# joaobuibergen/roms-trunk-mgh

Hardware: AMD Instinct MI355X
Metric: simulated-days/wall-sec (higher is better)
Workload: dtype f64; 1 GPU; BENCHMARK3 2048x256x30 NT=2 nonlinear 3-D step incl. 59 step2d calls, U3/C4 tracer advection, analytic atmospheric forcing, bulk fluxes + KPP + diagnostics every step; tiling=1x1, halo_transport=none, rccl_ranks=0, graph_exchanges=1, ndtfast=20, finite=True

## Files before the change

roms_trunk_mgh_amd/csrc/k_step2d_mom.hip:

```cpp
#include "step2d_common.h"

namespace {

enum { RM_pm = 0, RM_pn, RM_on_u, RM_om_v, RM_fomn, RM_dndx, RM_dmde, RM_pmon_r, RM_pnom_r, RM_pmon_p, RM_pnom_p,
       RM_om_r, RM_on_r, RM_om_p, RM_on_p,
       RM_h, RM_visc2_r, RM_visc2_p, RM_COUNT };
#define RM_FIRST_GROUP RM_h

typedef const double __attribute__((address_space(4))) *ccd_t;
template <bool ROWM>
struct Met {
  ccd_t tab;
  int nj, LBj;
  __device__ __forceinline__ double get(gcd_t A, int f, long q, int jr) const
  {
    if constexpr (ROWM) return tab[(jr - LBj) * RM_COUNT + f];
    else return A[q];
  }
};
#define MT(name, q, jr) met.get((gcd_t)c->F.name, RM_##name, (q), (jr))
#define HT(name, q, jr) meth.get((gcd_t)c->F.name, RM_##name, (q), (jr))

#define C6 (1.0 / 6.0)

struct T2 {
  const double *ub, *vb, *DU, *DV, *D;
  int i0, j0;
  int Istr, Iend, Jstr, Jend;
  bool s_edge, n_edge, w_edge, e_edge;
  __device__ __forceinline__ int at(int i, int j) const { return (i - i0) + (j - j0) * TP; }
};

__device__ __forceinline__ double UFx2(const T2 &m, int i, int j)
{
  int ia = i, ib = i + 1;
  if (m.w_edge) { if (ia == m.Istr) ia = m.Istr + 1; if (ib == m.Istr) ib = m.Istr + 1; }
  if (m.e_edge) { if (ia == m.Iend + 1) ia = m.Iend; if (ib == m.Iend + 1) ib = m.Iend; }
  const int a = m.at(i, j);
  return 0.25 * (m.ub[a] + m.ub[a + 1] - C6 * (d2x(m.ub, m.at(ia, j)) + d2x(m.ub, m.at(ib, j)))) *
         (m.DU[a] + m.DU[a + 1] - C6 * (d2x(m.DU, m.at(ia, j)) + d2x(m.DU, m.at(ib, j))));
}
__device__ __forceinline__ double UFe2(const T2 &m, int i, int j)
{
  int ja = j, jb = j - 1;
  if (m.s_edge) { if (ja == m.Jstr - 1) ja = m.Jstr; if (jb == m.Jstr - 1) jb = m.Jstr; }
  if (m.n_edge) { if (ja == m.Jend + 1) ja = m.Jend; if (jb == m.Jend + 1) jb = m.Jend; }
  const int a = m.at(i, j);
  return 0.25 * (m.ub[a] + m.ub[a - TP] - C6 * (d2y(m.ub, m.at(i, ja)) + d2y(m.ub, m.at(i, jb)))) *
         (m.DV[a] + m.DV[a - 1] - C6 * (d2x(m.DV, a) + d2x(m.DV, a - 1)));
}
__device__ __forceinline__ double VFx2(const T2 &m, int i, int j)
{
  int ia = i, ib = i - 1;
  if (m.w_edge) { if (ia == m.Istr - 1) ia = m.Istr; if (ib == m.Istr - 1) ib = m.Istr; }
  if (m.e_edge) { if (ia == m.Iend + 1) ia = m.Iend; if (ib == m.Iend + 1) ib = m.Iend; }
  const int a = m.at(i, j);
  return 0.25 * (m.vb[a] + m.vb[a - 1] - C6 * (d2x(m.vb, m.at(ia, j)) + d2x(m.vb, m.at(ib, j)))) *
         (m.DU[a] + m.DU[a - TP] - C6 * (d2y(m.DU, a) + d2y(m.DU, a - TP)));
}
__device__ __forceinline__ double VFe2(const T2 &m, int i, int j)
{
  int ja = j, jb = j + 1;
  if (m.s_edge) { if (ja == m.Jstr) ja = m.Jstr + 1; if (jb == m.Jstr) jb = m.Jstr + 1; }
  if (m.n_edge) { if (ja == m.Jend + 1) ja = m.Jend; if (jb == m.Jend + 1) jb = m.Jend; }
  const int a = m.at(i, j);
  return 0.25 * (m.vb[a] + m.vb[a + TP] - C6 * (d2y(m.vb, m.at(i, ja)) + d2y(m.vb, m.at(i, jb)))) *
         (m.DV[a] + m.DV[a + TP] - C6 * (d2y(m.DV, m.at(i, ja)) + d2y(m.DV, m.at(i, jb))));
}

__device__ __forceinline__ double UFx2_c2(const T2 &m, int a) { return 0.25 * (m.DU[a] + m.DU[a + 1]) * (m.ub[a] + m.ub[a + 1]); }
__device__ __forceinline__ double UFe2_c2(const T2 &m, int a) { return 0.25 * (m.DV[a] + m.DV[a - 1]) * (m.ub[a] + m.ub[a - TP]); }
__device__ __forceinline__ double VFx2_c2(const T2 &m, int a) { return 0.25 * (m.DU[a] + m.DU[a - TP]) * (m.vb[a] + m.vb[a - 1]); }
__device__ __forceinline__ double VFe2_c2(const T2 &m, int a) { return 0.25 * (m.DV[a] + m.DV[a + TP]) * (m.vb[a] + m.vb[a + TP]); }

template <bool FUSED, bool ROWM = false, bool ROWH = false, bool WET = false, bool C2 = false>
__global__ void __launch_bounds__(BLK_X *BLK_Y)
k2d_mom_lds(const RomsDev *__restrict__ c, S2 s, const double *__restrict__ DUon, const double *__restrict__ DVom,
            const double *__restrict__ zeta_new, const double *__restrict__ zwrk, double *__restrict__ DUnext,
            double *__restrict__ DVnext)
{
  DEV_PROLOGUE(c)
  const roms_params_t &p = c->p;
  const Met<ROWM> met{(ccd_t)c->rowm, (int)nj, LBj};
  const Met<ROWH> meth{(ccd_t)c->rowm, (int)nj, LBj};
  __shared__ double sU[TJ * TP], sV[TJ * TP], sDU[TJ * TP], sDV[TJ * TP], sD[TJ * TP];
  __shared__ double sZn[FUSED ? TJ * TP : 1], sZw[FUSED ? TJ * TP : 1];
  const bool img = FUSED && s.ew_images;
  const bool inline_bc = img || DUnext != nullptr;
  const Blk XB = xcd_block();
  const int i0 = b.Istr + XB.x * BLK_X, j0 = b.Jstr + XB.y * BLK_Y;
  static_assert(BLK_X == 64, "one wave per tile row");
  const int i = i0 + threadIdx.x, j = j0 + __builtin_amdgcn_readfirstlane(threadIdx.y);
  const gcd_t ubk = (gcd_t)(c->F.ubar + (long)(s.krhs - 1) * nij);
  const gcd_t vbk = (gcd_t)(c->F.vbar + (long)(s.krhs - 1) * nij);
  const gcd_t zk = (gcd_t)(c->F.zeta + (long)(s.krhs - 1) * nij);
  constexpr int ZW = BLK_X + 1, ZH = BLK_Y + 1;
  constexpr int ZIT = (ZW * ZH + BLK_X * BLK_Y - 1) / (BLK_X * BLK_Y);
  double z_zs[ZIT], z_zk[ZIT], z_rk[ZIT], z_rp[ZIT], z_rm[ZIT];
  double q_rhoA0 = 0.0, q_rhoS0 = 0.0, q_rhoAw = 0.0, q_rhoSw = 0.0, q_rhoAs = 0.0, q_rhoSs = 0.0;
  double q_zs0 = 0.0, q_zsw = 0.0, q_zss = 0.0, q_ruf = 0.0, q_rvf = 0.0, q_us = 0.0, q_vs = 0.0;
  double q_rubk = 0.0, q_rubp = 0.0, q_rvbk = 0.0, q_rvbp = 0.0;
  double q_Zt = 0.0, q_DU1 = 0.0, q_DU2 = 0.0, q_DV1 = 0.0, q_DV2 = 0.0, q_zkr = 0.0;
  if constexpr (FUSED) {
    const int tid = threadIdx.y * BLK_X + threadIdx.x;
    const gcd_t zsq = (gcd_t)(c->F.zeta + (long)(s.kstp - 1) * nij);
    const bool am3z = !(s.iif == 1 || s.predictor);
#pragma unroll
    for (int r = 0; r < ZIT; r++) {
      const int q = tid + r * BLK_X * BLK_Y;
      z_zs[r] = 0.0; z_zk[r] = 0.0; z_rk[r] = 0.0; z_rp[r] = 0.0; z_rm[r] = 1.0;
      if (q < ZW * ZH) {
        const int li = 1 + q % ZW, lj = 1 + q / ZW;
        int gi = i0 - 2 + li, gj = j0 - 2 + lj;
        if (img) gi = wrap_i(b, gi);
        else gi = gi < b.LBi ? b.LBi : (gi > b.UBi ? b.UBi : gi);
        gj = gj < b.LBj ? b.LBj : (gj > b.UBj ? b.UBj : gj);
        const long gq = I2(gi, gj);
        z_zs[r] = zsq[gq];
        z_zk[r] = zk[gq];
        if (am3z) {
          z_rk[r] = GF(rzeta)[gq + (long)(s.kstp - 1) * nij];
          z_rp[r] = GF(rzeta)[gq + (long)(3 - s.kstp - 1) * nij];
        }
        if (p.masking) z_rm[r] = GF(rmask)[gq];
      }
    }
    if (i <= b.Iend && j <= b.Jend) {
      const long a = I2(i, j);
      const gcd_t rhoA = (gcd_t)(c->F.rhoA), rhoS = (gcd_t)(c->F.rhoS);
      q_rhoA0 = rhoA[a]; q_rhoS0 = rhoS[a]; q_rhoAw = rhoA[a - 1]; q_rhoSw = rhoS[a - 1];
      q_rhoAs = rhoA[a - ni]; q_rhoSs = rhoS[a - ni];
      q_zs0 = zsq[a]; q_zsw = zsq[a - 1]; q_zss = zsq[a - ni];
      q_ruf = GF(rufrc)[a]; q_rvf = GF(rvfrc)[a];
      q_us = GF(ubar)[a + (long)(s.kstp - 1) * nij]; q_vs = GF(vbar)[a + (long)(s.kstp - 1) * nij];
      if (am3z) {
        q_rubk = GF(rubar)[a + (long)(s.kstp - 1) * nij]; q_rubp = GF(rubar)[a + (long)(3 - s.kstp - 1) * nij];
        q_rvbk = GF(rvbar)[a + (long)(s.kstp - 1) * nij]; q_rvbp = GF(rvbar)[a + (long)(3 - s.kstp - 1) * nij];
      }
      if (avg_reads_sums2(s)) { q_DU2 = GF(DU_avg2)[a]; q_DV2 = GF(DV_avg2)[a]; }
      if (avg_reads_sums1(s)) { q_Zt = GF(Zt_avg1)[a]; q_DU1 = GF(DU_avg1)[a]; q_DV1 = GF(DV_avg1)[a]; q_zkr = zk[a]; }
    }
  }
  {
    const int tid = threadIdx.y * BLK_X + threadIdx.x;
    for (int e = tid; e < TJ * TP; e += BLK_X * BLK_Y) {
      const int li = e % TP, lj = e / TP;
      int gi = i0 - 2 + li, gj = j0 - 2 + lj;
      if (img) gi = wrap_i(b, gi);
      else gi = gi < b.LBi ? b.LBi : (gi > b.UBi ? b.UBi : gi);
      gj = gj < b.LBj ? b.LBj : (gj > b.UBj ? b.UBj : gj);
      const long g = I2(gi, gj);
      const double ug = ubk[g], vg = vbk[g], Dg = zk[g] + HT(h, g, gj);
      sU[e] = ug;
      sV[e] = vg;
      sD[e] = Dg;
      if (DUon) {
        sDU[e] = DUon[g];
        sDV[e] = DVom[g];
      } else {
        sDU[e] = flux_u(ug, MT(on_u, g, gj), Dg, zk[g - 1] + HT(h, g - 1, gj));
        if (gj >= b.LBj + 1) sDV[e] = flux_v(vg, MT(om_v, g, gj), Dg, zk[g - ni] + HT(h, g - ni, gj - 1));
        else sDV[e] = 0.0;
      }
    }
  }
  __syncthreads();
  if constexpr (FUSED) {
    const int tid = threadIdx.y * BLK_X + threadIdx.x;
#pragma unroll
    for (int r = 0; r < ZIT; r++) {
      const int q = tid + r * BLK_X * BLK_Y;
      if (q < ZW * ZH) {
        const int li = 1 + q % ZW, lj = 1 + q / ZW;
        const int e = lj * TP + li;
        int gi = i0 - 2 + li, gj = j0 - 2 + lj;
        if (img) gi = wrap_i(b, gi);
        else gi = gi < b.LBi ? b.LBi : (gi > b.UBi ? b.UBi : gi);
        gj = gj < b.LBj ? b.LBj : (gj > b.UBj ? b.UBj : gj);
        const double rhs = (sDU[e] - sDU[e + 1]) + (sDV[e] - sDV[e + TP]);
        double zn, zw;
        const long gq = I2(gi, gj);
        zeta_step(p, s, rhs, MT(pm, gq, gj), MT(pn, gq, gj), z_zs[r], z_zk[r], z_rk[r], z_rp[r], z_rm[r],
                  p.masking != 0, zn, zw);
        sZn[e] = zn;
        sZw[e] = zw;
      }
    }
    __syncthreads();
  }
  if (i > b.Iend || j > b.Jend) return;
  auto put = [&](gd_t A, long idx, double val) {
    A[idx] = val;
    if (img) {
      if (i <= b.NghostPoints) A[idx + b.Lm] = val;
      if (i >= b.Lm - 2) A[idx - b.Lm] = val;
    }
  };
  const bool do_u = img || i >= b.IstrU;
  const bool do_v = j >= b.JstrV;
  const long a = I2(i, j);
  const gcd_t rhoA = (gcd_t)(c->F.rhoA);
  const gcd_t rhoS = (gcd_t)(c->F.rhoS);
  const gcd_t zs = (gcd_t)(c->F.zeta + (long)(s.kstp - 1) * nij);
  T2 m;
  m.ub = sU; m.vb = sV; m.DU = sDU; m.DV = sDV; m.D = sD;
  m.i0 = i0 - 2; m.j0 = j0 - 2;
  m.Istr = b.Istr; m.Iend = b.Iend; m.Jstr = b.Jstr; m.Jend = b.Jend;
  m.s_edge = b.south_edge && !b.NSperiodic; m.n_edge = b.north_edge && !b.NSperiodic;
  m.w_edge = b.west_edge && !b.EWperiodic;  m.e_edge = b.east_edge && !b.EWperiodic;
  const int t = m.at(i, j);
  const double fac = 1000.0 / p.rho0;
  const bool masking = p.masking != 0;
  auto mk = [&](gd_t M, long q) { return masking ? (double)M[q] : 1.0; };
  if constexpr (FUSED) {
    if (i >= b.IstrR && i <= b.IendR) {
      const bool inU = i >= b.Istr;
      store_average(c, s, a, inU, true,
                    fast_average(p, s, FastAvg{q_Zt, q_DU1, q_DU2, q_DV1, q_DV2}, sDU[t], sDV[t], q_zkr));
      if (j == b.Jstr && b.JstrR < b.Jstr) average_point(c, s, a - ni, inU, false, sDU[t - TP], sDV[t - TP], nij);
      if (j == b.Jend && b.JendR > b.Jend) average_point(c, s, a + ni, inU, true, sDU[t + TP], sDV[t + TP], nij);
    }
    const double zn = sZn[t];
    const gd_t zout = (gd_t)(c->F.zeta + (long)(s.knew - 1) * nij);
    put(zout, a, zn);
    if (b.south_edge && j == b.Jstr) put(zout, a - ni, masking ? zn * GF(rmask)[a - ni] : zn);
    if (b.north_edge && j == b.Jend) put(zout, a + ni, masking ? zn * GF(rmask)[a + ni] : zn);
    if (s.predictor)
      put((gd_t)(c->F.rzeta + (long)(s.krhs - 1) * nij), a, (sDU[t] - sDU[t + 1]) + (sDV[t] - sDV[t + TP]));
  }
  const double h0 = HT(h, a, j), hw = HT(h, a - 1, j), hs = HT(h, a - ni, j - 1);
  const double zw0 = FUSED ? sZw[t] : zwrk[a];
  const double rS0 = FUSED ? q_rhoS0 : (double)rhoS[a], rA0 = FUSED ? q_rhoA0 : (double)rhoA[a];
  const double gz0 = (fac + rS0) * zw0, gz20 = gz0 * zw0, gsa0 = zw0 * (rS0 - rA0);
  const double cg = 0.5 * p.g, c3 = 1.0 / 3.0;
  double rhs_u = 0.0, rhs_v = 0.0;
  if (do_u) {
    const long q = a - 1;
    const double zw = FUSED ? sZw[t - 1] : zwrk[q];
    const double rSq = FUSED ? q_rhoSw : (double)rhoS[q], rAq = FUSED ? q_rhoAw : (double)rhoA[q];
    const double gz = (fac + rSq) * zw, gz2 = gz * zw, gsa = zw * (rSq - rAq);
    rhs_u = cg * MT(on_u, a, j) *
            ((hw + h0) * (gz - gz0) +
             (hw - h0) * (gsa + gsa0 + c3 * (rAq - rA0) * (zw - zw0)) +
             (gz2 - gz20));
  }
  if (do_v) {
    const long q = a - ni;
    const double zw = FUSED ? sZw[t - TP] : zwrk[q];
    const double rSq = FUSED ? q_rhoSs : (double)rhoS[q], rAq = FUSED ? q_rhoAs : (double)rhoA[q];
    const double gz = (fac + rSq) * zw, gz2 = gz * zw, gsa = zw * (rSq - rAq);
    rhs_v = cg * MT(om_v, a, j) *
            ((hs + h0) * (gz - gz0) +
             (hs - h0) * (gsa + gsa0 + c3 * (rAq - rA0) * (zw - zw0)) +
             (gz2 - gz20));
  }
  if (p.uv_adv) {
    if constexpr (C2) {
      if (do_u) {
        const double cff1 = UFx2_c2(m, t) - UFx2_c2(m, t - 1);
        const double cff2 = UFe2_c2(m, t + TP) - UFe2_c2(m, t);
        rhs_u = rhs_u - (cff1 + cff2);
      }
      if (do_v) {
        const double cff1 = VFx2_c2(m, t + 1) - VFx2_c2(m, t);
        const double cff2 = VFe2_c2(m, t) - VFe2_c2(m, t - TP);
        rhs_v = rhs_v - (cff1 + cff2);
      }
    } else {
    if (do_u) {
      const double cff1 = UFx2(m, i, j) - UFx2(m, i - 1, j);
      const double cff2 = UFe2(m, i, j + 1) - UFe2(m, i, j);
      rhs_u = rhs_u - (cff1 + cff2);
    }
    if (do_v) {
      const double cff1 = VFx2(m, i + 1, j) - VFx2(m, i, j);
      const double cff2 = VFe2(m, i, j) - VFe2(m, i, j - 1);
      rhs_v = rhs_v - (cff1 + cff2);
    }
    }
  }
  const double D0 = sD[t], Dw = sD[t - 1], Ds = sD[t - TP];
  if (p.uv_cor) {
    const double cf0 = 0.5 * D0 * MT(fomn, a, j);
    const double UFx0 = cf0 * (sV[t] + sV[t + TP]);
    const double VFe0 = cf0 * (sU[t] + sU[t + 1]);
    if (do_u) {
      const double cfw = 0.5 * Dw * MT(fomn, a - 1, j);
      const double UFxw = cfw * (sV[t - 1] + sV[t - 1 + TP]);
      rhs_u = rhs_u + 0.5 * (UFx0 + UFxw);
    }
    if (do_v) {
      const double cfs = 0.5 * Ds * MT(fomn, a - ni, j - 1);
      const double VFes = cfs * (sU[t - TP] + sU[t - TP + 1]);
      rhs_v = rhs_v - 0.5 * (VFe0 + VFes);
    }
  }
  if (p.curvgrid && p.uv_adv) {
    auto cell = [&](long q, int jq, int tq, double D, double &ufx, double &vfe) {
      const double cff1 = 0.5 * (sV[tq] + sV[tq + TP]);
      const double cff2 = 0.5 * (sU[tq] + sU[tq + 1]);
      const double cff3 = cff1 * MT(dndx, q, jq);
      const double cff4 = cff2 * MT(dmde, q, jq);
      const double cff = D * (cff3 - cff4);
      ufx = cff * cff1;
      vfe = cff * cff2;
    };
    double u0, v0, u1, v1;
    cell(a, j, t, D0, u0, v0);
    if (do_u) { cell(a - 1, j, t - 1, Dw, u1, v1); rhs_u = rhs_u + 0.5 * (u0 + u1); }
    if (do_v) { cell(a - ni, j - 1, t - TP, Ds, u1, v1); rhs_v = rhs_v - 0.5 * (v0 + v1); }
  }
  if (p.uv_vis2) {
    auto str_r = [&](long q, int jq, int tq) {
      return HT(visc2_r, q, jq) * sD[tq] * 0.5 *
             (MT(pmon_r, q, jq) * ((MT(pn, q, jq) + MT(pn, q + 1, jq)) * sU[tq + 1] - (MT(pn, q - 1, jq) + MT(pn, q, jq)) * sU[tq]) -
              MT(pnom_r, q, jq) * ((MT(pm, q, jq) + MT(pm, q + ni, jq + 1)) * sV[tq + TP] - (MT(pm, q - ni, jq - 1) + MT(pm, q, jq)) * sV[tq]));
    };
    auto str_p = [&](long q, int jq, int tq) {
      const double Dp = 0.25 * (sD[tq] + sD[tq - 1] + sD[tq - TP] + sD[tq - 1 - TP]);
      const double cffp = HT(visc2_p, q, jq) * Dp * 0.5 *
             (MT(pmon_p, q, jq) * ((MT(pn, q - ni, jq - 1) + MT(pn, q, jq)) * sV[tq] - (MT(pn, q - 1 - ni, jq - 1) + MT(pn, q - 1, jq)) * sV[tq - 1]) +
              MT(pnom_p, q, jq) * ((MT(pm, q - 1, jq) + MT(pm, q, jq)) * sU[tq] - (MT(pm, q - 1 - ni, jq - 1) + MT(pm, q - ni, jq - 1)) * sU[tq - TP]));
      if constexpr (WET) return (masking ? cffp * GF(pmask)[q] : cffp) * GF(pmask_wet)[q];
      return masking ? cffp * GF(pmask)[q] : cffp;
    };
    const double sr0 = str_r(a, j, t), sp0 = str_p(a, j, t);
    if (do_u) {
      const double srw = str_r(a - 1, j, t - 1), spn = str_p(a + ni, j + 1, t + TP);
      const double onr0 = MT(on_r, a, j), onrw = MT(on_r, a - 1, j), omp0 = MT(om_p, a, j), ompn = MT(om_p, a + ni, j + 1);
      const double UFx0 = onr0 * onr0 * sr0, UFxw = onrw * onrw * srw;
      const double UFe0 = omp0 * omp0 * sp0, UFen = ompn * ompn * spn;
      const double cff1 = 0.5 * (MT(pn, a - 1, j) + MT(pn, a, j)) * (UFx0 - UFxw);
      const double cff2 = 0.5 * (MT(pm, a - 1, j) + MT(pm, a, j)) * (UFen - UFe0);
      rhs_u = rhs_u + (cff1 + cff2);
    }
    if (do_v) {
      const double srs = str_r(a - ni, j - 1, t - TP), spe = str_p(a + 1, j, t + 1);
      const double onp0 = MT(on_p, a, j), onpe = MT(on_p, a + 1, j), omr0 = MT(om_r, a, j), omrs = MT(om_r, a - ni, j - 1);
      const double VFx0 = onp0 * onp0 * sp0, VFxe = onpe * onpe * spe;
      const double VFe0 = omr0 * omr0 * sr0, VFes = omrs * omrs * srs;
      const double cff1 = 0.5 * (MT(pn, a - ni, j - 1) + MT(pn, a, j)) * (VFxe - VFx0);
      const double cff2 = 0.5 * (MT(pm, a - ni, j - 1) + MT(pm, a, j)) * (VFe0 - VFes);
      rhs_v = rhs_v + (cff1 - cff2);
    }
  }
  if (p.uv_vis4) {
    if (do_u) rhs_u = rhs_u - c->ws2[22][a];
    if (do_v) rhs_v = rhs_v - c->ws2[23][a];
  }
  if (c->clima.m2) {
    const gcd_t cof = (gcd_t)c->clima.M2nudgcof;
    if (do_u) {
      const double cff = 0.25 * (cof[a - 1] + cof[a]) * GF(om_u)[a] * MT(on_u, a, j);
      rhs_u = rhs_u + cff * (Dw + D0) * (((gcd_t)c->clima.ubarclm)[a] - sU[t]);
    }
    if (do_v) {
      const double cff = 0.25 * (cof[a - ni] + cof[a]) * MT(om_v, a, j) * GF(on_v)[a];
      rhs_v = rhs_v + cff * (Ds + D0) * (((gcd_t)c->clima.vbarclm)[a] - sV[t]);
    }
  }
  double rf_u = 0.0, rf_v = 0.0;
  if (s.iif == 1 && s.predictor) {
    const gd_t ru_s = (gd_t)(c->F.ru + (long)(s.nstp - 1) * n3w);
    const gd_t rv_s = (gd_t)(c->F.rv + (long)(s.nstp - 1) * n3w);
    const gcd_t ru_n = (gcd_t)(c->F.ru + (long)(s.nnew - 1) * n3w);
    const gcd_t rv_n = (gcd_t)(c->F.rv + (long)(s.nnew - 1) * n3w);
    if (do_u) {
      const double rf = (FUSED ? q_ruf : (double)GF(rufrc)[a]) - rhs_u;
      if (s.iic == s.ntfirst) rhs_u = rhs_u + rf;
      else if (s.iic == s.ntfirst + 1) rhs_u = rhs_u + 1.5 * rf - 0.5 * ru_n[a];
      else rhs_u = rhs_u + (23.0 / 12.0) * rf - (16.0 / 12.0) * ru_n[a] + (5.0 / 12.0) * ru_s[a];
      GF(rufrc)[a] = rf;
      ru_s[a] = rf;
      rf_u = rf;
    }
    if (do_v) {
      const double rf = (FUSED ? q_rvf : (double)GF(rvfrc)[a]) - rhs_v;
      if (s.iic == s.ntfirst) rhs_v = rhs_v + rf;
      else if (s.iic == s.ntfirst + 1) rhs_v = rhs_v + 1.5 * rf - 0.5 * rv_n[a];
      else rhs_v = rhs_v + (23.0 / 12.0) * rf - (16.0 / 12.0) * rv_n[a] + (5.0 / 12.0) * rv_s[a];
      GF(rvfrc)[a] = rf;
      rv_s[a] = rf;
      rf_v = rf;
    }
  } else {
    if (do_u) rhs_u = rhs_u + (FUSED ? q_ruf : (double)GF(rufrc)[a]);
    if (do_v) rhs_v = rhs_v + (FUSED ? q_rvf : (double)GF(rvfrc)[a]);
  }
  const double dtfast = p.dtfast;
  const double Dn0 = (FUSED ? sZn[t] : zeta_new[a]) + h0, Dst0 = (FUSED ? q_zs0 : (double)zs[a]) + h0;
  const int ptsk = 3 - s.kstp;
  const bool am3 = !(s.iif == 1 || s.predictor);
  const double c1 = (s.iif == 1) ? 0.5 * dtfast : dtfast;
  const double a1 = 0.5 * dtfast * 5.0 / 12.0, a2 = 0.5 * dtfast * 8.0 / 12.0, a3 = 0.5 * dtfast * 1.0 / 12.0;
  const gd_t ubn = (gd_t)(c->F.ubar + (long)(s.knew - 1) * nij);
  const gd_t vbn = (gd_t)(c->F.vbar + (long)(s.knew - 1) * nij);
  if (do_u) {
    const long q = a - 1;
    const double cff = (MT(pm, a, j) + MT(pm, q, j)) * (MT(pn, a, j) + MT(pn, q, j));
    const double fc = 1.0 / (Dn0 + ((FUSED ? sZn[t - 1] : zeta_new[q]) + hw));
    const double us = FUSED ? q_us : (double)GF(ubar)[a + (long)(s.kstp - 1) * nij];
    const double zsq = FUSED ? q_zsw : (double)zs[q];
    double un;
    if (!am3) un = (us * (Dst0 + (zsq + hw)) + cff * c1 * rhs_u) * fc;
    else un = (us * (Dst0 + (zsq + hw)) +
               cff * (a1 * rhs_u + a2 * (FUSED ? q_rubk : (double)GF(rubar)[a + (long)(s.kstp - 1) * nij]) -
                      a3 * (FUSED ? q_rubp : (double)GF(rubar)[a + (long)(ptsk - 1) * nij]))) * fc;
    if (masking) un = un * GF(umask)[a];
    if constexpr (WET) {
      const double cff7 = wet_factor(GF(umask_wet)[a], un);
      un = un * cff7;
      rhs_u = rhs_u * cff7;
      if (s.iif == 1 && s.predictor) {
        const double rf = rf_u * cff7;
        GF(rufrc)[a] = rf;
        ((gd_t)(c->F.ru + (long)(s.nstp - 1) * n3w))[a] = rf;
      }
    }
    put(ubn, a, un);
    if (s.predictor) GF(rubar)[a + (long)(s.krhs - 1) * nij] = rhs_u;
    const double un_s = masking ? (p.gamma2 * un) * GF(umask)[a - ni] : p.gamma2 * un;
    const double un_n = masking ? (p.gamma2 * un) * GF(umask)[a + ni] : p.gamma2 * un;
    if (inline_bc) {
      if (b.south_edge && j == b.Jstr) put(ubn, a - ni, un_s);
      if (b.north_edge && j == b.Jend) put(ubn, a + ni, un_n);
    }
    if constexpr (FUSED) {
      if (DUnext) {
        const double znw = sZn[t - 1];
        DUnext[a] = flux_u(un, MT(on_u, a, j), Dn0, znw + hw);
        if (b.south_edge && j == b.Jstr)
          DUnext[a - ni] = flux_u(un_s, MT(on_u, a - ni, j - 1), sZn[t] * mk(GF(rmask), a - ni) + hs,
                                  znw * mk(GF(rmask), q - ni) + HT(h, q - ni, j - 1));
        if (b.north_edge && j == b.Jend)
          DUnext[a + ni] = flux_u(un_n, MT(on_u, a + ni, j + 1), sZn[t] * mk(GF(rmask), a + ni) + HT(h, a + ni, j + 1),
                                  znw * mk(GF(rmask), q + ni) + HT(h, q + ni, j + 1));
      }
    }
  }
  if (do_v) {
    const long q = a - ni;
    const double cff = (MT(pm, a, j) + MT(pm, q, j - 1)) * (MT(pn, a, j) + MT(pn, q, j - 1));
    const double fc = 1.0 / (Dn0 + ((FUSED ? sZn[t - TP] : zeta_new[q]) + hs));
    const double vs = FUSED ? q_vs : (double)GF(vbar)[a + (long)(s.kstp - 1) * nij];
    const double zsq = FUSED ? q_zss : (double)zs[q];
    double vn;
    if (!am3) vn = (vs * (Dst0 + (zsq + hs)) + cff * c1 * rhs_v) * fc;
    else vn = (vs * (Dst0 + (zsq + hs)) +
               cff * (a1 * rhs_v + a2 * (FUSED ? q_rvbk : (double)GF(rvbar)[a + (long)(s.kstp - 1) * nij]) -
                      a3 * (FUSED ? q_rvbp : (double)GF(rvbar)[a + (long)(ptsk - 1) * nij]))) * fc;
    if (masking) vn = vn * GF(vmask)[a];
    if constexpr (WET) {
      const double cff7 = wet_factor(GF(vmask_wet)[a], vn);
      vn = vn * cff7;
      rhs_v = rhs_v * cff7;
      if (s.iif == 1 && s.predictor) {
        const double rf = rf_v * cff7;
        GF(rvfrc)[a] = rf;
        ((gd_t)(c->F.rv + (long)(s.nstp - 1) * n3w))[a] = rf;
      }
    }
    put(vbn, a, vn);
    if (s.predictor) GF(rvbar)[a + (long)(s.krhs - 1) * nij] = rhs_v;
    if constexpr (FUSED) {
      if (DVnext) DVnext[a] = flux_v(vn, MT(om_v, a, j), Dn0, sZn[t - TP] + hs);
    }
  }
  if (inline_bc) {
    if (b.south_edge && j == b.Jstr) put(vbn, a, 0.0);
    if (b.north_edge && j == b.Jend) put(vbn, a + ni, 0.0);
  }
  if constexpr (FUSED) {
    if (DVnext) {
      const double zn0 = sZn[t];
      if (b.south_edge && j == b.Jstr)
        DVnext[a] = flux_v(0.0, MT(om_v, a, j), zn0 + h0, zn0 * mk(GF(rmask), a - ni) + hs);
      if (b.north_edge && j == b.Jend)
        DVnext[a + ni] = flux_v(0.0, MT(om_v, a + ni, j + 1), zn0 * mk(GF(rmask), a + ni) + HT(h, a + ni, j + 1), zn0 + h0);
    }
  }
}

__global__ void k_rowm_build(const RomsDev *__restrict__ c, double *__restrict__ tab, int *__restrict__ flag)
{
  DEV_PROLOGUE(c)
  const int jr = blockIdx.x, f = blockIdx.y;
  const double *const A[RM_COUNT] = {c->F.pm, c->F.pn, c->F.on_u, c->F.om_v, c->F.fomn, c->F.dndx, c->F.dmde,
                                     c->F.pmon_r, c->F.pnom_r, c->F.pmon_p, c->F.pnom_p, c->F.om_r, c->F.on_r,
                                     c->F.om_p, c->F.on_p, c->F.h, c->F.visc2_r, c->F.visc2_p};
  const double *a = A[f];
  if (!a) {
    if (threadIdx.x == 0) tab[(long)jr * RM_COUNT + f] = 0.0;
    return;
  }
  const int ng = b.NghostPoints;
  const int i0 = (b.Istr - ng > b.LBi) ? b.Istr - ng : b.LBi, i1 = (b.Iend + ng < b.UBi) ? b.Iend + ng : b.UBi;
  const unsigned long long *row = reinterpret_cast<const unsigned long long *>(a + (long)jr * ni) - LBi;
  const unsigned long long v0 = row[b.Istr];
  bool differs = false;
  for (int i = i0 + (int)threadIdx.x; i <= i1; i += (int)blockDim.x) differs |= row[i] != v0;
  if (differs) atomicOr(flag + (f >= RM_FIRST_GROUP ? 1 : 0), 1);
  if (threadIdx.x == 0) tab[(long)jr * RM_COUNT + f] = a[(long)jr * ni + (b.Istr - LBi)];
}

}

extern "C" int roms_hip_row_metrics_state(void) { return g_ctx.rowm_state == 1 && g_ctx.rowh ? 3 : g_ctx.rowm_state; }

bool roms_rowm_is_table_field(int id)
{
  static const int ids[RM_COUNT] = {FID_pm, FID_pn, FID_on_u, FID_om_v, FID_fomn, FID_dndx, FID_dmde, FID_pmon_r,
                                    FID_pnom_r, FID_pmon_p, FID_pnom_p, FID_om_r, FID_on_r, FID_om_p, FID_on_p,
                                    FID_h, FID_visc2_r, FID_visc2_p};
  for (int q = 0; q < RM_COUNT; q++)
    if (ids[q] == id) return true;
  return false;
}

void roms_rowm_invalidate()
{
  if (g_ctx.rowm_state) step2d_graphs_release();
  g_ctx.rowm_state = 0;
}

void roms_rowm_release()
{
  if (g_ctx.rowm_dev) (void)hipFree(g_ctx.rowm_dev);
  g_ctx.rowm_dev = nullptr;
  g_ctx.rowm_nj = 0;
  g_ctx.rowm_state = 0;
  g_ctx.hostc.rowm = nullptr;
}

int roms_rowm_prepare()
{
  if (g_ctx.rowm_state) return 0;
  const roms_bounds_t &b = g_ctx.b;
  const long nj = b.UBj - b.LBj + 1;
  if (g_ctx.rowm_nj != nj) {
    roms_rowm_release();
    HIP_TRY(hipMalloc(&g_ctx.rowm_dev, sizeof(double) * (RM_COUNT * nj + 1)));
    g_ctx.rowm_nj = nj;
  }
  int *flag = reinterpret_cast<int *>(g_ctx.rowm_dev + RM_COUNT * nj);
  int rc = roms_flush_consts();
  if (rc) return rc;
  HIP_TRY(hipMemsetAsync(flag, 0, sizeof(double), g_ctx.stream));
  hipLaunchKernelGGL(k_rowm_build, dim3((unsigned)nj, RM_COUNT), dim3(256), 0, g_ctx.stream, g_ctx.devc,
                     g_ctx.rowm_dev, flag);
  KERNEL_CHECK("k_rowm_build");
  int differs[2] = {0, 0};
  HIP_TRY(hipMemcpyAsync(differs, flag, 2 * sizeof(int), hipMemcpyDeviceToHost, g_ctx.stream));
  HIP_TRY(hipStreamSynchronize(g_ctx.stream));
  g_ctx.rowm_state = differs[0] ? 2 : 1;
  g_ctx.rowh = !differs[0] && !differs[1];
  const double *want = differs[0] ? nullptr : g_ctx.rowm_dev;
  if (g_ctx.hostc.rowm != want) {
    g_ctx.hostc.rowm = want;
    g_ctx.devc_dirty = true;
    if ((rc = roms_flush_consts())) return rc;
  }
  return 0;
}

template <bool FUSED>
static auto pick_k2d(bool c2, bool rowm, bool rowh, bool wet) -> decltype(&k2d_mom_lds<FUSED, false, false, false, false>)
{
  if constexpr (!FUSED) {
    if (wet) return c2 ? k2d_mom_lds<false, false, false, true, true> : k2d_mom_lds<false, false, false, true, false>;
    return c2 ? k2d_mom_lds<false, false, false, false, true> : k2d_mom_lds<false, false, false, false, false>;
  } else {
    if (rowh) return c2 ? k2d_mom_lds<true, true, true, false, true> : k2d_mom_lds<true, true, true, false, false>;
    if (rowm) return c2 ? k2d_mom_lds<true, true, false, false, true> : k2d_mom_lds<true, true, false, false, false>;
    return c2 ? k2d_mom_lds<true, false, false, false, true> : k2d_mom_lds<true, false, false, false, false>;
  }
}

int roms_launch_k2d_mom_lds(const S2 &s, K2dLaunch mode, const double *DUon, const double *DVom, const double *zeta_new,
                            const double *zwrk, double *DUnext, double *DVnext)
{
  const roms_bounds_t &b = g_ctx.b;
  const bool rowm = g_ctx.rowm_state == 1, rowh = rowm && g_ctx.rowh;
  const bool c2 = g_ctx.p.uv_adv && ROMS_UV_HADV(g_ctx.p.uv_adv) == ROMS_UVH_C2;
  const bool wet = g_ctx.p.wet_dry != 0;
  const auto kernel = mode == K2dLaunch::Split ? pick_k2d<false>(c2, false, false, wet)
                                               : pick_k2d<true>(c2, rowm, rowh, false);
  hipLaunchKernelGGL(kernel, grid2d(b.Iend - b.Istr + 1, b.Jend - b.Jstr + 1), block2d(), 0, g_ctx.stream, g_ctx.devc, s,
                     DUon, DVom, zeta_new, zwrk, DUnext, DVnext);
  KERNEL_CHECK("k2d_mom_lds");
  return 0;
}
```

Before: 0.2301 simulated-days/s.

## Precompute derived row-metric sums/products and restructure zeta halo point mapping

Extends the per-row metric table with precomputed derived quantities (pm/pn pair sums, squared on/om metrics, half-sums, and the cff products) built by a new derive kernel, so the viscosity and momentum update paths read one constant-cache entry instead of several and do less arithmetic. The zeta halo computation now uses a fixed two-iteration mapping, one interior row per wave plus an extra row and column, instead of div/mod index decoding. Edge predicates are computed per workgroup to cut redundant checks. The derived-table entries lean on row-invariance and neighbouring-row assumptions that must hold exactly, and the new halo mapping has to cover every point the old one did.

```diff
diff --git a/roms_trunk_mgh_amd/csrc/k_step2d_mom.hip b/roms_trunk_mgh_amd/csrc/k_step2d_mom.hip
--- a/roms_trunk_mgh_amd/csrc/k_step2d_mom.hip
+++ b/roms_trunk_mgh_amd/csrc/k_step2d_mom.hip
@@ -4,7 +4,18 @@
 
 enum { RM_pm = 0, RM_pn, RM_on_u, RM_om_v, RM_fomn, RM_dndx, RM_dmde, RM_pmon_r, RM_pnom_r, RM_pmon_p, RM_pnom_p,
        RM_om_r, RM_on_r, RM_om_p, RM_on_p,
-       RM_h, RM_visc2_r, RM_visc2_p, RM_COUNT };
+       RM_h, RM_visc2_r, RM_visc2_p, RM_ARRAYS,
+       RM_pn2 = RM_ARRAYS,
+       RM_pm2,
+       RM_pm_n,
+       RM_pm_s,
+       RM_pn_s,
+       RM_on_r2, RM_om_r2, RM_on_p2, RM_om_p2,
+       RM_hpn2, RM_hpm2,
+       RM_hpn_s, RM_hpm_s,
+       RM_cff_u,
+       RM_cff_v,
+       RM_COUNT };
 #define RM_FIRST_GROUP RM_h
 
 typedef const double __attribute__((address_space(4))) *ccd_t;
@@ -12,14 +23,38 @@
 struct Met {
   ccd_t tab;
   int nj, LBj;
+  __device__ __forceinline__ double col(int f, int jr) const { return tab[(jr - LBj) * RM_COUNT + f]; }
   __device__ __forceinline__ double get(gcd_t A, int f, long q, int jr) const
   {
-    if constexpr (ROWM) return tab[(jr - LBj) * RM_COUNT + f];
+    if constexpr (ROWM) return col(f, jr);
     else return A[q];
+  }
+  __device__ __forceinline__ double sum(gcd_t A, long q1, long q2, int fd, int jr) const
+  {
+    if constexpr (ROWM) return col(fd, jr);
+    else return A[q1] + A[q2];
+  }
+  __device__ __forceinline__ double hsum(gcd_t A, long q1, long q2, int fd, int jr) const
+  {
+    if constexpr (ROWM) return col(fd, jr);
+    else return 0.5 * (A[q1] + A[q2]);
+  }
+  __device__ __forceinline__ double sqr(gcd_t A, long q, int fd, int jr) const
+  {
+    if constexpr (ROWM) return col(fd, jr);
+    else { const double x = A[q]; return x * x; }
+  }
+  __device__ __forceinline__ double sumprod(gcd_t A, gcd_t B, long q1, long q2, int fd, int jr) const
+  {
+    if constexpr (ROWM) return col(fd, jr);
+    else return (A[q1] + A[q2]) * (B[q1] + B[q2]);
   }
 };
 #define MT(name, q, jr) met.get((gcd_t)c->F.name, RM_##name, (q), (jr))
 #define HT(name, q, jr) meth.get((gcd_t)c->F.name, RM_##name, (q), (jr))
+#define MSUM(name, q1, q2, DER, jr) met.sum((gcd_t)c->F.name, (q1), (q2), RM_##DER, (jr))
+#define MHSUM(name, q1, q2, DER, jr) met.hsum((gcd_t)c->F.name, (q1), (q2), RM_##DER, (jr))
+#define MSQR(name, q, jr) met.sqr((gcd_t)c->F.name, (q), RM_##name##2, (jr))
 
 #define C6 (1.0 / 6.0)
 
@@ -95,27 +130,36 @@
   const gcd_t vbk = (gcd_t)(c->F.vbar + (long)(s.krhs - 1) * nij);
   const gcd_t zk = (gcd_t)(c->F.zeta + (long)(s.krhs - 1) * nij);
   constexpr int ZW = BLK_X + 1, ZH = BLK_Y + 1;
-  constexpr int ZIT = (ZW * ZH + BLK_X * BLK_Y - 1) / (BLK_X * BLK_Y);
+  constexpr int ZIT = 2;
   double z_zs[ZIT], z_zk[ZIT], z_rk[ZIT], z_rp[ZIT], z_rm[ZIT];
+  const int tx = threadIdx.x, wy = __builtin_amdgcn_readfirstlane(threadIdx.y);
+  const int gj_last = b.UBj;
+  auto clamp_j = [&](int gj) { return gj < LBj ? LBj : (gj > gj_last ? gj_last : gj); };
+  auto clamp_i = [&](int gi) {
+    if (img) return wrap_i(b, gi);
+    return gi < b.LBi ? b.LBi : (gi > b.UBi ? b.UBi : gi);
+  };
+  const bool z_col = wy == 1;
+  struct ZPoint { bool on; int e, gj; long gq; };
+  auto zpoint = [&](const int r) {
+    const bool col = r == 1 && z_col;
+    const int li = col ? ZW : 1 + tx, lj = r == 0 ? 1 + wy : (col ? 1 + tx : ZH);
+    const int gj = clamp_j(j0 - 2 + lj);
+    return ZPoint{r == 0 || wy == 0 || (col && tx < ZH), lj * TP + li, gj, I2(clamp_i(i0 - 2 + li), gj)};
+  };
   double q_rhoA0 = 0.0, q_rhoS0 = 0.0, q_rhoAw = 0.0, q_rhoSw = 0.0, q_rhoAs = 0.0, q_rhoSs = 0.0;
   double q_zs0 = 0.0, q_zsw = 0.0, q_zss = 0.0, q_ruf = 0.0, q_rvf = 0.0, q_us = 0.0, q_vs = 0.0;
   double q_rubk = 0.0, q_rubp = 0.0, q_rvbk = 0.0, q_rvbp = 0.0;
   double q_Zt = 0.0, q_DU1 = 0.0, q_DU2 = 0.0, q_DV1 = 0.0, q_DV2 = 0.0, q_zkr = 0.0;
   if constexpr (FUSED) {
-    const int tid = threadIdx.y * BLK_X + threadIdx.x;
     const gcd_t zsq = (gcd_t)(c->F.zeta + (long)(s.kstp - 1) * nij);
     const bool am3z = !(s.iif == 1 || s.predictor);
 #pragma unroll
     for (int r = 0; r < ZIT; r++) {
-      const int q = tid + r * BLK_X * BLK_Y;
       z_zs[r] = 0.0; z_zk[r] = 0.0; z_rk[r] = 0.0; z_rp[r] = 0.0; z_rm[r] = 1.0;
-      if (q < ZW * ZH) {
-        const int li = 1 + q % ZW, lj = 1 + q / ZW;
-        int gi = i0 - 2 + li, gj = j0 - 2 + lj;
-        if (img) gi = wrap_i(b, gi);
-        else gi = gi < b.LBi ? b.LBi : (gi > b.UBi ? b.UBi : gi);
-        gj = gj < b.LBj ? b.LBj : (gj > b.UBj ? b.UBj : gj);
-        const long gq = I2(gi, gj);
+      const ZPoint z = zpoint(r);
+      if (z.on) {
+        const long gq = z.gq;
         z_zs[r] = zsq[gq];
         z_zk[r] = zk[gq];
         if (am3z) {
@@ -166,22 +210,20 @@
   }
   __syncthreads();
   if constexpr (FUSED) {
-    const int tid = threadIdx.y * BLK_X + threadIdx.x;
 #pragma unroll
     for (int r = 0; r < ZIT; r++) {
-      const int q = tid + r * BLK_X * BLK_Y;
-      if (q < ZW * ZH) {
-        const int li = 1 + q % ZW, lj = 1 + q / ZW;
-        const int e = lj * TP + li;
-        int gi = i0 - 2 + li, gj = j0 - 2 + lj;
-        if (img) gi = wrap_i(b, gi);
-        else gi = gi < b.LBi ? b.LBi : (gi > b.UBi ? b.UBi : gi);
-        gj = gj < b.LBj ? b.LBj : (gj > b.UBj ? b.UBj : gj);
+      const ZPoint z = zpoint(r);
+      if (z.on) {
+        const int e = z.e;
         const double rhs = (sDU[e] - sDU[e + 1]) + (sDV[e] - sDV[e + TP]);
-        double zn, zw;
-        const long gq = I2(gi, gj);
-        zeta_step(p, s, rhs, MT(pm, gq, gj), MT(pn, gq, gj), z_zs[r], z_zk[r], z_rk[r], z_rp[r], z_rm[r],
-                  p.masking != 0, zn, zw);
+        double zn, zw, pm_a, pn_a;
+        if (r == 1 && z_col) {
+          pm_a = MT(pm, z.gq, z.gj); pn_a = MT(pn, z.gq, z.gj);
+        } else {
+          const int gjs = clamp_j(j0 - 2 + (r == 0 ? 1 + wy : ZH));
+          pm_a = MT(pm, z.gq, gjs); pn_a = MT(pn, z.gq, gjs);
+        }
+        zeta_step(p, s, rhs, pm_a, pn_a, z_zs[r], z_zk[r], z_rk[r], z_rp[r], z_rm[r], p.masking != 0, zn, zw);
         sZn[e] = zn;
         sZw[e] = zw;
       }
@@ -206,8 +248,11 @@
   m.ub = sU; m.vb = sV; m.DU = sDU; m.DV = sDV; m.D = sD;
   m.i0 = i0 - 2; m.j0 = j0 - 2;
   m.Istr = b.Istr; m.Iend = b.Iend; m.Jstr = b.Jstr; m.Jend = b.Jend;
-  m.s_edge = b.south_edge && !b.NSperiodic; m.n_edge = b.north_edge && !b.NSperiodic;
-  m.w_edge = b.west_edge && !b.EWperiodic;  m.e_edge = b.east_edge && !b.EWperiodic;
+  const bool wg_s = b.south_edge && j0 == b.Jstr, wg_n = b.north_edge && j0 + BLK_Y > b.Jend;
+  const bool wg_w = b.west_edge && i0 == b.Istr, wg_e = b.east_edge && i0 + BLK_X > b.Iend;
+  const bool at_s = wg_s && j == b.Jstr, at_n = wg_n && j == b.Jend;
+  m.s_edge = wg_s && !b.NSperiodic; m.n_edge = wg_n && !b.NSperiodic;
+  m.w_edge = wg_w && !b.EWperiodic;  m.e_edge = wg_e && !b.EWperiodic;
   const int t = m.at(i, j);
   const double fac = 1000.0 / p.rho0;
   const bool masking = p.masking != 0;
@@ -223,8 +268,8 @@
     const double zn = sZn[t];
     const gd_t zout = (gd_t)(c->F.zeta + (long)(s.knew - 1) * nij);
     put(zout, a, zn);
-    if (b.south_edge && j == b.Jstr) put(zout, a - ni, masking ? zn * GF(rmask)[a - ni] : zn);
-    if (b.north_edge && j == b.Jend) put(zout, a + ni, masking ? zn * GF(rmask)[a + ni] : zn);
+    if (at_s) put(zout, a - ni, masking ? zn * GF(rmask)[a - ni] : zn);
+    if (at_n) put(zout, a + ni, masking ? zn * GF(rmask)[a + ni] : zn);
     if (s.predictor)
       put((gd_t)(c->F.rzeta + (long)(s.krhs - 1) * nij), a, (sDU[t] - sDU[t + 1]) + (sDV[t] - sDV[t + TP]));
   }
@@ -313,34 +358,32 @@
   if (p.uv_vis2) {
     auto str_r = [&](long q, int jq, int tq) {
       return HT(visc2_r, q, jq) * sD[tq] * 0.5 *
-             (MT(pmon_r, q, jq) * ((MT(pn, q, jq) + MT(pn, q + 1, jq)) * sU[tq + 1] - (MT(pn, q - 1, jq) + MT(pn, q, jq)) * sU[tq]) -
-              MT(pnom_r, q, jq) * ((MT(pm, q, jq) + MT(pm, q + ni, jq + 1)) * sV[tq + TP] - (MT(pm, q - ni, jq - 1) + MT(pm, q, jq)) * sV[tq]));
+             (MT(pmon_r, q, jq) * (MSUM(pn, q, q + 1, pn2, jq) * sU[tq + 1] - MSUM(pn, q - 1, q, pn2, jq) * sU[tq]) -
+              MT(pnom_r, q, jq) * (MSUM(pm, q, q + ni, pm_n, jq) * sV[tq + TP] - MSUM(pm, q - ni, q, pm_s, jq) * sV[tq]));
     };
     auto str_p = [&](long q, int jq, int tq) {
       const double Dp = 0.25 * (sD[tq] + sD[tq - 1] + sD[tq - TP] + sD[tq - 1 - TP]);
       const double cffp = HT(visc2_p, q, jq) * Dp * 0.5 *
-             (MT(pmon_p, q, jq) * ((MT(pn, q - ni, jq - 1) + MT(pn, q, jq)) * sV[tq] - (MT(pn, q - 1 - ni, jq - 1) + MT(pn, q - 1, jq)) * sV[tq - 1]) +
-              MT(pnom_p, q, jq) * ((MT(pm, q - 1, jq) + MT(pm, q, jq)) * sU[tq] - (MT(pm, q - 1 - ni, jq - 1) + MT(pm, q - ni, jq - 1)) * sU[tq - TP]));
+             (MT(pmon_p, q, jq) * (MSUM(pn, q - ni, q, pn_s, jq) * sV[tq] - MSUM(pn, q - 1 - ni, q - 1, pn_s, jq) * sV[tq - 1]) +
+              MT(pnom_p, q, jq) * (MSUM(pm, q - 1, q, pm2, jq) * sU[tq] - MSUM(pm, q - 1 - ni, q - ni, pm2, jq - 1) * sU[tq - TP]));
       if constexpr (WET) return (masking ? cffp * GF(pmask)[q] : cffp) * GF(pmask_wet)[q];
       return masking ? cffp * GF(pmask)[q] : cffp;
     };
     const double sr0 = str_r(a, j, t), sp0 = str_p(a, j, t);
     if (do_u) {
       const double srw = str_r(a - 1, j, t - 1), spn = str_p(a + ni, j + 1, t + TP);
-      const double onr0 = MT(on_r, a, j), onrw = MT(on_r, a - 1, j), omp0 = MT(om_p, a, j), ompn = MT(om_p, a + ni, j + 1);
-      const double UFx0 = onr0 * onr0 * sr0, UFxw = onrw * onrw * srw;
-      const double UFe0 = omp0 * omp0 * sp0, UFen = ompn * ompn * spn;
-      const double cff1 = 0.5 * (MT(pn, a - 1, j) + MT(pn, a, j)) * (UFx0 - UFxw);
-      const double cff2 = 0.5 * (MT(pm, a - 1, j) + MT(pm, a, j)) * (UFen - UFe0);
+      const double UFx0 = MSQR(on_r, a, j) * sr0, UFxw = MSQR(on_r, a - 1, j) * srw;
+      const double UFe0 = MSQR(om_p, a, j) * sp0, UFen = MSQR(om_p, a + ni, j + 1) * spn;
+      const double cff1 = MHSUM(pn, a - 1, a, hpn2, j) * (UFx0 - UFxw);
+      const double cff2 = MHSUM(pm, a - 1, a, hpm2, j) * (UFen - UFe0);
       rhs_u = rhs_u + (cff1 + cff2);
     }
     if (do_v) {
       const double srs = str_r(a - ni, j - 1, t - TP), spe = str_p(a + 1, j, t + 1);
-      const double onp0 = MT(on_p, a, j), onpe = MT(on_p, a + 1, j), omr0 = MT(om_r, a, j), omrs = MT(om_r, a - ni, j - 1);
-      const double VFx0 = onp0 * onp0 * sp0, VFxe = onpe * onpe * spe;
-      const double VFe0 = omr0 * omr0 * sr0, VFes = omrs * omrs * srs;
-      const double cff1 = 0.5 * (MT(pn, a - ni, j - 1) + MT(pn, a, j)) * (VFxe - VFx0);
-      const double cff2 = 0.5 * (MT(pm, a - ni, j - 1) + MT(pm, a, j)) * (VFe0 - VFes);
+      const double VFx0 = MSQR(on_p, a, j) * sp0, VFxe = MSQR(on_p, a + 1, j) * spe;
+      const double VFe0 = MSQR(om_r, a, j) * sr0, VFes = MSQR(om_r, a - ni, j - 1) * srs;
+      const double cff1 = MHSUM(pn, a - ni, a, hpn_s, j) * (VFxe - VFx0);
+      const double cff2 = MHSUM(pm, a - ni, a, hpm_s, j) * (VFe0 - VFes);
       rhs_v = rhs_v + (cff1 - cff2);
     }
   }
@@ -397,7 +440,7 @@
   const gd_t vbn = (gd_t)(c->F.vbar + (long)(s.knew - 1) * nij);
   if (do_u) {
     const long q = a - 1;
-    const double cff = (MT(pm, a, j) + MT(pm, q, j)) * (MT(pn, a, j) + MT(pn, q, j));
+    const double cff = met.sumprod((gcd_t)c->F.pm, (gcd_t)c->F.pn, a, q, RM_cff_u, j);
     const double fc = 1.0 / (Dn0 + ((FUSED ? sZn[t - 1] : zeta_new[q]) + hw));
     const double us = FUSED ? q_us : (double)GF(ubar)[a + (long)(s.kstp - 1) * nij];
     const double zsq = FUSED ? q_zsw : (double)zs[q];
@@ -422,17 +465,17 @@
     const double un_s = masking ? (p.gamma2 * un) * GF(umask)[a - ni] : p.gamma2 * un;
     const double un_n = masking ? (p.gamma2 * un) * GF(umask)[a + ni] : p.gamma2 * un;
     if (inline_bc) {
-      if (b.south_edge && j == b.Jstr) put(ubn, a - ni, un_s);
-      if (b.north_edge && j == b.Jend) put(ubn, a + ni, un_n);
+      if (at_s) put(ubn, a - ni, un_s);
+      if (at_n) put(ubn, a + ni, un_n);
     }
     if constexpr (FUSED) {
       if (DUnext) {
         const double znw = sZn[t - 1];
         DUnext[a] = flux_u(un, MT(on_u, a, j), Dn0, znw + hw);
-        if (b.south_edge && j == b.Jstr)
+        if (at_s)
           DUnext[a - ni] = flux_u(un_s, MT(on_u, a - ni, j - 1), sZn[t] * mk(GF(rmask), a - ni) + hs,
                                   znw * mk(GF(rmask), q - ni) + HT(h, q - ni, j - 1));
-        if (b.north_edge && j == b.Jend)
+        if (at_n)
           DUnext[a + ni] = flux_u(un_n, MT(on_u, a + ni, j + 1), sZn[t] * mk(GF(rmask), a + ni) + HT(h, a + ni, j + 1),
                                   znw * mk(GF(rmask), q + ni) + HT(h, q + ni, j + 1));
       }
@@ -440,7 +483,7 @@
   }
   if (do_v) {
     const long q = a - ni;
-    const double cff = (MT(pm, a, j) + MT(pm, q, j - 1)) * (MT(pn, a, j) + MT(pn, q, j - 1));
+    const double cff = met.sumprod((gcd_t)c->F.pm, (gcd_t)c->F.pn, a, q, RM_cff_v, j);
     const double fc = 1.0 / (Dn0 + ((FUSED ? sZn[t - TP] : zeta_new[q]) + hs));
     const double vs = FUSED ? q_vs : (double)GF(vbar)[a + (long)(s.kstp - 1) * nij];
     const double zsq = FUSED ? q_zss : (double)zs[q];
@@ -467,15 +510,15 @@
     }
   }
   if (inline_bc) {
-    if (b.south_edge && j == b.Jstr) put(vbn, a, 0.0);
-    if (b.north_edge && j == b.Jend) put(vbn, a + ni, 0.0);
+    if (at_s) put(vbn, a, 0.0);
+    if (at_n) put(vbn, a + ni, 0.0);
   }
   if constexpr (FUSED) {
     if (DVnext) {
       const double zn0 = sZn[t];
-      if (b.south_edge && j == b.Jstr)
+      if (at_s)
         DVnext[a] = flux_v(0.0, MT(om_v, a, j), zn0 + h0, zn0 * mk(GF(rmask), a - ni) + hs);
-      if (b.north_edge && j == b.Jend)
+      if (at_n)
         DVnext[a + ni] = flux_v(0.0, MT(om_v, a + ni, j + 1), zn0 * mk(GF(rmask), a + ni) + HT(h, a + ni, j + 1), zn0 + h0);
     }
   }
@@ -485,7 +528,7 @@
 {
   DEV_PROLOGUE(c)
   const int jr = blockIdx.x, f = blockIdx.y;
-  const double *const A[RM_COUNT] = {c->F.pm, c->F.pn, c->F.on_u, c->F.om_v, c->F.fomn, c->F.dndx, c->F.dmde,
+  const double *const A[RM_ARRAYS] = {c->F.pm, c->F.pn, c->F.on_u, c->F.om_v, c->F.fomn, c->F.dndx, c->F.dmde,
                                      c->F.pmon_r, c->F.pnom_r, c->F.pmon_p, c->F.pnom_p, c->F.om_r, c->F.on_r,
                                      c->F.om_p, c->F.on_p, c->F.h, c->F.visc2_r, c->F.visc2_p};
   const double *a = A[f];
@@ -503,16 +546,42 @@
   if (threadIdx.x == 0) tab[(long)jr * RM_COUNT + f] = a[(long)jr * ni + (b.Istr - LBi)];
 }
 
+__global__ void k_rowm_derive(double *__restrict__ tab, int nj)
+{
+  const int jr = blockIdx.x * blockDim.x + threadIdx.x;
+  if (jr >= nj) return;
+  double *const T = tab + (long)jr * RM_COUNT;
+  const bool has_s = jr > 0, has_n = jr + 1 < nj;
+  const double pm = T[RM_pm], pn = T[RM_pn];
+  const double pm_s = has_s ? T[RM_pm - RM_COUNT] : 0.0, pn_s = has_s ? T[RM_pn - RM_COUNT] : 0.0;
+  const double pm_n = has_n ? T[RM_pm + RM_COUNT] : 0.0;
+  T[RM_pn2] = pn + pn;
+  T[RM_pm2] = pm + pm;
+  T[RM_pm_n] = has_n ? pm + pm_n : 0.0;
+  T[RM_pm_s] = has_s ? pm_s + pm : 0.0;
+  T[RM_pn_s] = has_s ? pn_s + pn : 0.0;
+  T[RM_on_r2] = T[RM_on_r] * T[RM_on_r];
+  T[RM_om_r2] = T[RM_om_r] * T[RM_om_r];
+  T[RM_on_p2] = T[RM_on_p] * T[RM_on_p];
+  T[RM_om_p2] = T[RM_om_p] * T[RM_om_p];
+  T[RM_hpn2] = 0.5 * (pn + pn);
+  T[RM_hpm2] = 0.5 * (pm + pm);
+  T[RM_hpn_s] = has_s ? 0.5 * (pn_s + pn) : 0.0;
+  T[RM_hpm_s] = has_s ? 0.5 * (pm_s + pm) : 0.0;
+  T[RM_cff_u] = (pm + pm) * (pn + pn);
+  T[RM_cff_v] = has_s ? (pm + pm_s) * (pn + pn_s) : 0.0;
+}
+
 }
 
 extern "C" int roms_hip_row_metrics_state(void) { return g_ctx.rowm_state == 1 && g_ctx.rowh ? 3 : g_ctx.rowm_state; }
 
 bool roms_rowm_is_table_field(int id)
 {
-  static const int ids[RM_COUNT] = {FID_pm, FID_pn, FID_on_u, FID_om_v, FID_fomn, FID_dndx, FID_dmde, FID_pmon_r,
+  static const int ids[RM_ARRAYS] = {FID_pm, FID_pn, FID_on_u, FID_om_v, FID_fomn, FID_dndx, FID_dmde, FID_pmon_r,
                                     FID_pnom_r, FID_pmon_p, FID_pnom_p, FID_om_r, FID_on_r, FID_om_p, FID_on_p,
                                     FID_h, FID_visc2_r, FID_visc2_p};
-  for (int q = 0; q < RM_COUNT; q++)
+  for (int q = 0; q < RM_ARRAYS; q++)
     if (ids[q] == id) return true;
   return false;
 }
@@ -546,9 +615,11 @@
   int rc = roms_flush_consts();
   if (rc) return rc;
   HIP_TRY(hipMemsetAsync(flag, 0, sizeof(double), g_ctx.stream));
-  hipLaunchKernelGGL(k_rowm_build, dim3((unsigned)nj, RM_COUNT), dim3(256), 0, g_ctx.stream, g_ctx.devc,
+  hipLaunchKernelGGL(k_rowm_build, dim3((unsigned)nj, RM_ARRAYS), dim3(256), 0, g_ctx.stream, g_ctx.devc,
                      g_ctx.rowm_dev, flag);
   KERNEL_CHECK("k_rowm_build");
+  hipLaunchKernelGGL(k_rowm_derive, dim3((unsigned)((nj + 63) / 64)), dim3(64), 0, g_ctx.stream, g_ctx.rowm_dev, (int)nj);
+  KERNEL_CHECK("k_rowm_derive");
   int differs[2] = {0, 0};
   HIP_TRY(hipMemcpyAsync(differs, flag, 2 * sizeof(int), hipMemcpyDeviceToHost, g_ctx.stream));
   HIP_TRY(hipStreamSynchronize(g_ctx.stream));
```

Result: no change. 0.2300 simulated-days/s (median of 2 runs) (-0.1%).
